# TAMUparametric/PPOPT

Measured on AMD Instinct MI355X. Metric: candidate active-sets checked/sec (combinatorial mpQP), higher is better.
Workload: dtype f64

## Files before the change

ppopt_amd/csrc/kernels.hpp:

```cpp
#pragma once
#include <stdint.h>

#include "kkt.hpp"
#include "records.hpp"

#ifndef MPC_GLOBAL
#define MPC_GLOBAL __global__
#define MPC_LB(...) __launch_bounds__(__VA_ARGS__)
#endif

namespace mpc {

constexpr int ST_INFEASIBLE = 0, ST_FEASIBLE = 1, ST_OPT_NO_REGION = 2, ST_REGION = 3, ST_SINGULAR = 4, ST_LP_LIMIT = 5;
constexpr int ST_OPT_PENDING = 6;
constexpr int ST_RETRY = 7;
constexpr int ST_NEEDX = 8;
constexpr int ST_NEEDX_SING = 9;
static_assert(ST_REGION == SLOT_ST_REGION, "records.hpp: the status of a slot that carries a record");
constexpr double ZERO_ROW_ATOL = 1e-8;
constexpr double FULL_DIM_RADIUS = 1e-8;

struct DevProblem {
    int n_x, n_t, n_c, n_eq, n_tc, is_qp, kkt_mode;
    const double *A, *b, *F, *c, *H, *Q, *A_t, *b_t;
// ... 552 lines not shown
    if (lane == 63) wsum[w] = incl;
    __syncthreads();
    if (w == 0) {
        int t = lane < 16 ? wsum[lane] : 0, ti = t;
#pragma unroll
        for (int off = 1; off < 16; off <<= 1) { const int o = __shfl_up(ti, off); if (lane >= off) ti += o; }
        if (lane < 16) wsum[lane] = ti - t;
        if (lane == 15 && total_out) *total_out = ti;
    }
    __syncthreads();
    return incl - v + wsum[w];
}
constexpr int SCAN_IT = 4;
__device__ __forceinline__ void block_exclusive_scan_it(const int (&v)[SCAN_IT], int (&ex)[SCAN_IT], int *total_out) {
    constexpr int NW = 16 / SCAN_IT;
    __shared__ int wsum_it[NW];
    const int lane = threadIdx.x & 63, w = threadIdx.x >> 6;
    int s = 0;
#pragma unroll
    for (int k = 0; k < SCAN_IT; ++k) s += v[k];
    int incl = s;
#pragma unroll
    for (int off = 1; off < 64; off <<= 1) { const int o = __shfl_up(incl, off); if (lane >= off) incl += o; }
    if (lane == 63) wsum_it[w] = incl;
    __syncthreads();
    int base = 0;
#pragma unroll
    for (int k = 0; k < NW; ++k) base += k < w ? wsum_it[k] : 0;
    if (total_out && threadIdx.x == 64 * NW - 1) *total_out = base + incl;
    int run = base + incl - s;
#pragma unroll
    for (int k = 0; k < SCAN_IT; ++k) { ex[k] = run; run += v[k]; }
    __syncthreads();
}
MPC_GLOBAL void MPC_LB(1024 / SCAN_IT) k_scan_block_sums(const int32_t *__restrict__ in, long long n, int32_t *__restrict__ sums) {
    __shared__ int tot;
    const long long i0 = blockIdx.x * (long long)SCAN_BLOCK + (long long)threadIdx.x * SCAN_IT;
    int v[SCAN_IT], ex[SCAN_IT];
#pragma unroll
    for (int k = 0; k < SCAN_IT; ++k) v[k] = i0 + k < n ? in[i0 + k] : 0;
    block_exclusive_scan_it(v, ex, &tot);
    if (threadIdx.x == 0) sums[blockIdx.x] = tot;
}
MPC_GLOBAL void MPC_LB(1024 / SCAN_IT) k_scan_sums(int32_t *__restrict__ sums, int nb, int32_t *__restrict__ total) {
    __shared__ int tot;
    int carry = 0;
    for (int base = 0; base < nb; base += SCAN_BLOCK) {
        const int i0 = base + (int)threadIdx.x * SCAN_IT;
        int v[SCAN_IT], ex[SCAN_IT];
#pragma unroll
        for (int k = 0; k < SCAN_IT; ++k) v[k] = i0 + k < nb ? sums[i0 + k] : 0;
        block_exclusive_scan_it(v, ex, &tot);
#pragma unroll
        for (int k = 0; k < SCAN_IT; ++k) if (i0 + k < nb) sums[i0 + k] = ex[k] + carry;
        carry += tot;
        __syncthreads();
    }
    if (threadIdx.x == 0) *total = carry;
}
MPC_GLOBAL void MPC_LB(1024 / SCAN_IT) k_scan_apply(const int32_t *__restrict__ in, int32_t *__restrict__ out, long long n,
                                                    const int32_t *__restrict__ sums) {
    const long long i0 = blockIdx.x * (long long)SCAN_BLOCK + (long long)threadIdx.x * SCAN_IT;
    int v[SCAN_IT], ex[SCAN_IT];
#pragma unroll
    for (int k = 0; k < SCAN_IT; ++k) v[k] = i0 + k < n ? in[i0 + k] : 0;
    block_exclusive_scan_it(v, ex, nullptr);
    const int add = sums[blockIdx.x];
#pragma unroll
    for (int k = 0; k < SCAN_IT; ++k) if (i0 + k < n) out[i0 + k] = ex[k] + add;
}

constexpr int PART_CLASSES = 4;
__device__ __forceinline__ int part_class(unsigned long long spec, int st) { return (int)((spec >> (4 * (st & 15))) & 15ull); }
MPC_GLOBAL void MPC_LB(1024 / SCAN_IT) k_part_count(const uint8_t *__restrict__ status, long long n, unsigned long long spec,
                                                     int32_t *__restrict__ blockcounts, int nb) {
    constexpr int BT = 1024 / SCAN_IT, NW = BT / 64;
    __shared__ int wc[16][PART_CLASSES];
    const int wave = threadIdx.x >> 6, lane = threadIdx.x & 63;
#pragma unroll
    for (int j = 0; j < SCAN_IT; ++j) {
        const long long i = blockIdx.x * 1024LL + j * BT + threadIdx.x;
        const int cls = i < n ? part_class(spec, status[i]) : 15;
#pragma unroll
        for (int c = 0; c < PART_CLASSES; ++c) {
            const unsigned long long m = __ballot(cls == c);
            if (lane == 0) wc[j * NW + wave][c] = __popcll(m);
        }
    }
    __syncthreads();
    if (threadIdx.x < PART_CLASSES) {
        int tot = 0;
        for (int w = 0; w < 16; ++w) tot += wc[w][threadIdx.x];
        blockcounts[threadIdx.x * nb + blockIdx.x] = tot;
    }
}
MPC_GLOBAL void MPC_LB(1024 / SCAN_IT) k_part_sums(int32_t *__restrict__ blockcounts, int nb, int32_t *__restrict__ totals) {
    __shared__ int tot;
    int32_t *sums = blockcounts + (size_t)blockIdx.x * nb;
    int carry = 0;
    for (int base = 0; base < nb; base += SCAN_BLOCK) {
        const int i0 = base + (int)threadIdx.x * SCAN_IT;
        int v[SCAN_IT], ex[SCAN_IT];
#pragma unroll
        for (int k = 0; k < SCAN_IT; ++k) v[k] = i0 + k < nb ? sums[i0 + k] : 0;
        block_exclusive_scan_it(v, ex, &tot);
#pragma unroll
        for (int k = 0; k < SCAN_IT; ++k) if (i0 + k < nb) sums[i0 + k] = ex[k] + carry;
        carry += tot;
        __syncthreads();
    }
    if (threadIdx.x == 0) totals[blockIdx.x] = carry;
}
MPC_GLOBAL void MPC_LB(1024 / SCAN_IT) k_part_scatter(const uint8_t *__restrict__ status, long long n, unsigned long long spec,
                                                       const int32_t *__restrict__ blockbase, int nb, int32_t *__restrict__ lists) {
    constexpr int BT = 1024 / SCAN_IT, NW = BT / 64;
    __shared__ int wc[16][PART_CLASSES];
    const int wave = threadIdx.x >> 6, lane = threadIdx.x & 63;
    int cls[SCAN_IT], within[SCAN_IT];
#pragma unroll
    for (int j = 0; j < SCAN_IT; ++j) {
        const long long i = blockIdx.x * 1024LL + j * BT + threadIdx.x;
        cls[j] = i < n ? part_class(spec, status[i]) : 15;
        within[j] = 0;
#pragma unroll
        for (int c = 0; c < PART_CLASSES; ++c) {
            const unsigned long long m = __ballot(cls[j] == c);
            if (lane == 0) wc[j * NW + wave][c] = __popcll(m);
            if (cls[j] == c) within[j] = __popcll(m & ((1ull << lane) - 1ull));
        }
    }
    __syncthreads();
#pragma unroll
    for (int j = 0; j < SCAN_IT; ++j) {
        if (cls[j] < PART_CLASSES) {
            const long long i = blockIdx.x * 1024LL + j * BT + threadIdx.x;
            int before = 0;
            for (int w = 0; w < j * NW + wave; ++w) before += wc[w][cls[j]];
            lists[(size_t)cls[j] * n + blockbase[cls[j] * nb + blockIdx.x] + before + within[j]] = (int32_t)i;
        }
    }
}

MPC_GLOBAL void k_flag_status(const uint8_t *__restrict__ status, long long n, int lo, int hi, int32_t *__restrict__ flag) {
    const long long i = blockIdx.x * (long long)blockDim.x + threadIdx.x;
    if (i < n) flag[i] = status[i] >= lo && status[i] <= hi;
}
MPC_GLOBAL void k_scatter_index(const int32_t *__restrict__ flag, const int32_t *__restrict__ pos, long long n,
                                int32_t *__restrict__ list) {
    const long long i = blockIdx.x * (long long)blockDim.x + threadIdx.x;
    if (i < n && flag[i]) list[pos[i]] = (int32_t)i;
}

struct ZeroBufs { void *p[4]; unsigned long long bytes[4]; };
MPC_GLOBAL void MPC_LB(256) k_zero_bufs(ZeroBufs z) {
    for (int j = 0; j < 4; ++j) {
        const unsigned long long bytes = z.bytes[j];
        if (!z.p[j] || bytes == 0) continue;
        if ((reinterpret_cast<unsigned long long>(z.p[j]) & 7ull) == 0 && (bytes & 7ull) == 0) {
            unsigned long long *p = reinterpret_cast<unsigned long long *>(z.p[j]);
            for (unsigned long long i = blockIdx.x * 256ull + threadIdx.x; i < bytes / 8; i += (unsigned long long)gridDim.x * 256ull) p[i] = 0ull;
        } else {
            unsigned char *p = reinterpret_cast<unsigned char *>(z.p[j]);
            for (unsigned long long i = blockIdx.x * 256ull + threadIdx.x; i < bytes; i += (unsigned long long)gridDim.x * 256ull) p[i] = 0;
        }
    }
}

struct RegionPrep { ZeroBufs z; const int32_t *copy_src; int32_t *copy_dst; long long copy_n; int32_t *head_i; int fi, first, extra; };
MPC_GLOBAL void MPC_LB(256) k_region_prep(RegionPrep a) {
    for (int j = 0; j < 4; ++j) {
        const unsigned long long bytes = a.z.bytes[j];
        if (!a.z.p[j] || bytes == 0) continue;
        if ((reinterpret_cast<unsigned long long>(a.z.p[j]) & 7ull) == 0 && (bytes & 7ull) == 0) {
            unsigned long long *p = reinterpret_cast<unsigned long long *>(a.z.p[j]);
            for (unsigned long long i = blockIdx.x * 256ull + threadIdx.x; i < bytes / 8; i += (unsigned long long)gridDim.x * 256ull) p[i] = 0ull;
        } else {
            unsigned char *p = reinterpret_cast<unsigned char *>(a.z.p[j]);
            for (unsigned long long i = blockIdx.x * 256ull + threadIdx.x; i < bytes; i += (unsigned long long)gridDim.x * 256ull) p[i] = 0;
        }
    }
    for (long long i = blockIdx.x * 256ll + threadIdx.x; i < a.copy_n; i += (long long)gridDim.x * 256ll) a.copy_dst[i] = a.copy_src[i];
    for (int j = blockIdx.x * 256 + threadIdx.x; j < a.extra; j += gridDim.x * 256) { int32_t *hi = a.head_i + (size_t)(a.first + j) * a.fi; hi[SW_STATUS] = 0; hi[SW_CAND] = -1; }
}

struct FetchCopy { const void *src[3]; void *dst[3]; unsigned long long bytes[3]; unsigned int *counter; int32_t *flag; };
MPC_GLOBAL void MPC_LB(256) k_fetch_slots(FetchCopy a) {
    for (int j = 0; j < 3; ++j) {
        const unsigned long long words = a.bytes[j] / 4;
        const unsigned int *src = static_cast<const unsigned int *>(a.src[j]);
        unsigned int *dst = static_cast<unsigned int *>(a.dst[j]);
        for (unsigned long long i = blockIdx.x * 256ull + threadIdx.x; i < words; i += (unsigned long long)gridDim.x * 256ull) dst[i] = src[i];
    }
    __builtin_amdgcn_fence(__ATOMIC_RELEASE, "");
    __syncthreads();
    if (threadIdx.x == 0) {
        if (atomicAdd(a.counter, 1u) + 1u == gridDim.x) {
            __builtin_amdgcn_fence(__ATOMIC_ACQ_REL, "");
            atomicExch(a.counter, 0u);
            __hip_atomic_store(a.flag, 1, __ATOMIC_RELEASE, __HIP_MEMORY_SCOPE_SYSTEM);
        }
    }
}

struct FetchEntry { const void *src; void *dst; unsigned long long bytes; };
MPC_GLOBAL void MPC_LB(256) k_fetch_many(const FetchEntry *__restrict__ tab) {
    const FetchEntry e = tab[blockIdx.y];
    const unsigned long long words = e.bytes / 4;
    const unsigned int *src = static_cast<const unsigned int *>(e.src);
    unsigned int *dst = static_cast<unsigned int *>(e.dst);
    for (unsigned long long i = blockIdx.x * 256ull + threadIdx.x; i < words; i += (unsigned long long)gridDim.x * 256ull) dst[i] = src[i];
}

MPC_GLOBAL void k_publish_words(const unsigned int *__restrict__ src, unsigned int *__restrict__ dst, int n) {
    for (int i = threadIdx.x; i < n; i += blockDim.x) dst[i] = src[i];
}
MPC_GLOBAL void k_publish_words2(const unsigned int *__restrict__ src1, int n1, const unsigned int *__restrict__ src2, int n2, unsigned int *__restrict__ dst) {
    for (int i = threadIdx.x; i < n1 + n2; i += blockDim.x) dst[i] = i < n1 ? src1[i] : src2[i - n1];
}

constexpr int SMALL_LEVEL_N = 16384;
MPC_GLOBAL void MPC_LB(1024) k_compact_small(const uint8_t *__restrict__ status, int n, int lo, int hi,
                                                        int32_t *__restrict__ list, int32_t *__restrict__ total) {
    __shared__ int wc[16];
    __shared__ int base;
    const int wave = threadIdx.x >> 6, lane = threadIdx.x & 63;
    if (threadIdx.x == 0) base = 0;
    __syncthreads();
    for (int start = 0; start < n; start += 1024) {
        const int i = start + (int)threadIdx.x;
        const bool f = i < n && status[i] >= lo && status[i] <= hi;
        const unsigned long long m = __ballot(f);
        if (lane == 0) wc[wave] = __popcll(m);
        __syncthreads();
        int before = base;
        for (int w = 0; w < wave; ++w) before += wc[w];
        if (f) list[before + __popcll(m & ((1ull << lane) - 1ull))] = i;
        __syncthreads();
        if (threadIdx.x == 0) { int t = 0; for (int w = 0; w < 16; ++w) t += wc[w]; base += t; }
        __syncthreads();
    }
    if (threadIdx.x == 0) *total = base;
}
MPC_GLOBAL void MPC_LB(1024) k_partition_small(const uint8_t *__restrict__ status, int n, unsigned long long spec,
                                                          int32_t *__restrict__ lists, long long stride, int32_t *__restrict__ totals) {
    __shared__ int wc[16][PART_CLASSES];
    __shared__ int base[PART_CLASSES];
    const int wave = threadIdx.x >> 6, lane = threadIdx.x & 63;
    if (threadIdx.x < PART_CLASSES) base[threadIdx.x] = 0;
    __syncthreads();
    for (int start = 0; start < n; start += 1024) {
        const int i = start + (int)threadIdx.x;
        const int cls = i < n ? part_class(spec, status[i]) : 15;
        int within = 0;
#pragma unroll
        for (int c = 0; c < PART_CLASSES; ++c) {
            const unsigned long long m = __ballot(cls == c);
            if (lane == 0) wc[wave][c] = __popcll(m);
            if (cls == c) within = __popcll(m & ((1ull << lane) - 1ull));
        }
        __syncthreads();
        if (cls < PART_CLASSES) {
            int before = base[cls];
            for (int w = 0; w < wave; ++w) before += wc[w][cls];
            lists[(size_t)cls * stride + before + within] = i;
        }
        __syncthreads();
        if (threadIdx.x < PART_CLASSES) { int t = 0; for (int w = 0; w < 16; ++w) t += wc[w][threadIdx.x]; base[threadIdx.x] += t; }
        __syncthreads();
    }
    if (threadIdx.x < PART_CLASSES) totals[threadIdx.x] = base[threadIdx.x];
}
MPC_GLOBAL void MPC_LB(1024) k_scan_small(const int32_t *__restrict__ in, int32_t *__restrict__ out, int n,
                                                     int32_t *__restrict__ total) {
    __shared__ int tot;
    int carry = 0;
    for (int start = 0; start < n; start += SCAN_BLOCK) {
        const int i = start + (int)threadIdx.x;
        const int ex = block_exclusive_scan_1024(i < n ? in[i] : 0, &tot);
        __syncthreads();
        if (i < n) out[i] = ex + carry;
        carry += tot;
        __syncthreads();
    }
    if (threadIdx.x == 0) *total = carry;
}

constexpr int EXPAND_LOWDIM = 1, EXPAND_PENDING = 2;
__device__ __forceinline__ bool expands(int st, int keep_lowdim = 0) {
    return st == ST_FEASIBLE || st == ST_REGION || st == ST_SINGULAR || st == ST_LP_LIMIT || ((keep_lowdim & EXPAND_LOWDIM) && st == ST_OPT_NO_REGION) ||
           ((keep_lowdim & EXPAND_PENDING) && st == ST_OPT_PENDING);
}

template <int MW>
__device__ __forceinline__ void set_mask(const int32_t *as, int k, unsigned long long (&p)[MW]) {
#pragma unroll
    for (int w = 0; w < MW; ++w) p[w] = 0;
    for (int i = 0; i < k; ++i) {
        const int v = as[i];
#pragma unroll
        for (int w = 0; w < MW; ++w) if ((v >> 6) == w) p[w] |= 1ull << (v & 63);
    }
}

template <int MW>
MPC_GLOBAL void MPC_LB(64) k_children_count(DevProblem P, const int32_t *__restrict__ cands, long long n, int k,
                                                       const uint8_t *__restrict__ status,
                                                       const unsigned long long *__restrict__ pruned, long long n_pruned,
                                                       unsigned long long *__restrict__ childmask, int32_t *__restrict__ count, int keep_lowdim) {
    const long long c = blockIdx.x;
    const int lane = lane_id();
    if (c >= n) return;
    const int st = status[c];
    unsigned long long m[MW];
#pragma unroll
    for (int w = 0; w < MW; ++w) m[w] = 0;
    if (expands(st, keep_lowdim)) {
        const int32_t *as = cands + (size_t)c * k;
        unsigned long long p[MW], a[MW], kill[MW];
        set_mask<MW>(as, k, p);
        const int start = k > 0 ? as[k - 1] + 1 : 0;
        int stop = P.n_c;
        if (!P.is_qp && st == ST_FEASIBLE) stop = min(stop, (k + 1) + P.n_c - P.n_x);
#pragma unroll
        for (int w = 0; w < MW; ++w) {
            const int lo = max(start - 64 * w, 0), hi = min(stop - 64 * w, 64);
            a[w] = hi > lo ? ((hi >= 64 ? ~0ull : ((1ull << hi) - 1ull)) & ~((1ull << lo) - 1ull)) : 0ull;
            kill[w] = 0;
        }
        for (long long j = lane; j < n_pruned; j += 64) {
            unsigned long long d[MW];
            int bits = 0;
#pragma unroll
            for (int w = 0; w < MW; ++w) { d[w] = pruned[MW * j + w] & ~p[w]; bits += __popcll(d[w]); }
            if (bits == 0) {
#pragma unroll
                for (int w = 0; w < MW; ++w) kill[w] = ~0ull;
            } else if (bits == 1) {
#pragma unroll
                for (int w = 0; w < MW; ++w) kill[w] |= d[w];
            }
        }
#pragma unroll
        for (int w = 0; w < MW; ++w) {
            for (int off = 32; off > 0; off >>= 1) kill[w] |= __shfl_xor(kill[w], off);
            m[w] = a[w] & ~kill[w];
        }
    }
    if (lane == 0) {
        int cnt = 0;
#pragma unroll
        for (int w = 0; w < MW; ++w) { childmask[MW * c + w] = m[w]; cnt += __popcll(m[w]); }
        count[c] = cnt;
    }
}

constexpr int PB_OFF = 256, PB_CUR = 513, PB_SINGLES = 776, PB_WORDS = PB_SINGLES + 2 * 4;
template <int MW>
__device__ __forceinline__ int pruned_min_member(const unsigned long long *p, int ne, int *n_members) {
    int first = -1, cnt = 0;
#pragma unroll
    for (int w = 0; w < MW; ++w) {
        unsigned long long v = p[w];
        const int lo = ne - 64 * w;
        if (lo >= 64) v = 0ull; else if (lo > 0) v &= ~((1ull << lo) - 1ull);
        cnt += __popcll(v);
        if (first < 0 && v) first = 64 * w + __ffsll((long long)v) - 1;
    }
    *n_members = cnt;
    return first;
}
template <int MW>
MPC_GLOBAL void MPC_LB(256) k_pruned_bucket_count(const unsigned long long *__restrict__ pruned, long long n_pruned, int ne, int32_t *__restrict__ head) {
    const long long j = (long long)blockIdx.x * 256 + threadIdx.x;
    if (j >= n_pruned) return;
    int cnt = 0;
    const int b = pruned_min_member<MW>(pruned + (size_t)MW * j, ne, &cnt);
    if (cnt <= 1) {
        unsigned long long *singles = reinterpret_cast<unsigned long long *>(head + PB_SINGLES);
#pragma unroll
        for (int w = 0; w < MW; ++w) { const unsigned long long v = cnt == 0 ? ~0ull : pruned[(size_t)MW * j + w]; if (v) atomicOr(&singles[w], v); }
    } else if (b >= 0) atomicAdd(&head[b], 1);
}
MPC_GLOBAL void MPC_LB(256) k_pruned_bucket_scan(int32_t *__restrict__ head) {
    __shared__ int sh[256];
    const int t = threadIdx.x;
    sh[t] = head[t];
    __syncthreads();
    for (int off = 1; off < 256; off <<= 1) { const int v = t >= off ? sh[t - off] : 0; __syncthreads(); sh[t] += v; __syncthreads(); }
    head[PB_OFF + t + 1] = sh[t];
    if (t == 0) head[PB_OFF] = 0;
    head[PB_CUR + t] = 0;
}
template <int MW>
MPC_GLOBAL void MPC_LB(256) k_pruned_bucket_scatter(const unsigned long long *__restrict__ pruned, long long n_pruned, int ne, int32_t *__restrict__ head,
                                                            unsigned long long *__restrict__ out) {
    const long long j = (long long)blockIdx.x * 256 + threadIdx.x;
    if (j >= n_pruned) return;
    int cnt = 0;
    const int b = pruned_min_member<MW>(pruned + (size_t)MW * j, ne, &cnt);
    if (cnt <= 1 || b < 0) return;
    const int pos = head[PB_OFF + b] + atomicAdd(&head[PB_CUR + b], 1);
#pragma unroll
    for (int w = 0; w < MW; ++w) out[(size_t)MW * pos + w] = pruned[(size_t)MW * j + w];
}
template <int MW>
MPC_GLOBAL void MPC_LB(64) k_children_count_b(DevProblem P, const int32_t *__restrict__ cands, long long n, int k,
                                                         const uint8_t *__restrict__ status,
                                                         const unsigned long long *__restrict__ bucketed, const int32_t *__restrict__ head,
                                                         unsigned long long *__restrict__ childmask, int32_t *__restrict__ count, int keep_lowdim) {
    const long long c = blockIdx.x;
    const int lane = lane_id();
    if (c >= n) return;
    const int st = status[c];
    unsigned long long m[MW];
#pragma unroll
    for (int w = 0; w < MW; ++w) m[w] = 0;
    if (expands(st, keep_lowdim)) {
        const int32_t *as = cands + (size_t)c * k;
        unsigned long long p[MW], a[MW], kill[MW];
        set_mask<MW>(as, k, p);
        const int start = k > 0 ? as[k - 1] + 1 : 0;
        int stop = P.n_c;
        if (!P.is_qp && st == ST_FEASIBLE) stop = min(stop, (k + 1) + P.n_c - P.n_x);
        const unsigned long long *singles = reinterpret_cast<const unsigned long long *>(head + PB_SINGLES);
#pragma unroll
        for (int w = 0; w < MW; ++w) {
            const int lo = max(start - 64 * w, 0), hi = min(stop - 64 * w, 64);
            a[w] = hi > lo ? ((hi >= 64 ? ~0ull : ((1ull << hi) - 1ull)) & ~((1ull << lo) - 1ull)) : 0ull;
            kill[w] = singles[w] & ~p[w];
            const int lo_e = P.n_eq - 64 * w;
            const unsigned long long emask = lo_e >= 64 ? ~0ull : (lo_e > 0 ? ((1ull << lo_e) - 1ull) : 0ull);
            if (singles[w] & p[w] & ~emask) kill[w] = ~0ull;
        }
        for (int mi = P.n_eq; mi < k; ++mi) {
            const int b = as[mi];
            const int j0 = head[PB_OFF + b], j1 = head[PB_OFF + b + 1];
            for (int j = j0 + lane; j < j1; j += 64) {
                unsigned long long d[MW];
                int bits = 0;
#pragma unroll
                for (int w = 0; w < MW; ++w) { d[w] = bucketed[(size_t)MW * j + w] & ~p[w]; bits += __popcll(d[w]); }
                if (bits == 0) {
#pragma unroll
                    for (int w = 0; w < MW; ++w) kill[w] = ~0ull;
                } else if (bits == 1) {
#pragma unroll
                    for (int w = 0; w < MW; ++w) kill[w] |= d[w];
                }
            }
        }
#pragma unroll
        for (int w = 0; w < MW; ++w) {
            for (int off = 32; off > 0; off >>= 1) kill[w] |= __shfl_xor(kill[w], off);
            m[w] = a[w] & ~kill[w];
        }
    }
    if (lane == 0) {
        int cnt = 0;
#pragma unroll
        for (int w = 0; w < MW; ++w) { childmask[MW * c + w] = m[w]; cnt += __popcll(m[w]); }
        count[c] = cnt;
    }
}

MPC_GLOBAL void MPC_LB(64) k_children_write(const int32_t *__restrict__ cands, long long n, int k, int mw,
                                                       const unsigned long long *__restrict__ childmask,
                                                       const int32_t *__restrict__ offset, int32_t *__restrict__ out,
                                                       const uint8_t *__restrict__ stored, int32_t *__restrict__ parent_slot) {
    const long long c = blockIdx.x;
    const int lane = lane_id();
    if (c >= n) return;
    const int32_t *as = cands + (size_t)c * k;
    int base = offset[c];
    const int ps = (stored && stored[c]) ? (int)c : -1;
    for (int half = 0; half < mw; ++half) {
        const unsigned long long mk = childmask[(size_t)mw * c + half];
        if (!mk) continue;
        const bool mine = (mk >> lane) & 1ull;
        const int pos = base + __popcll(mk & ((1ull << lane) - 1ull));
        if (mine) {
            int32_t *o = out + (size_t)pos * (k + 1);
            for (int i = 0; i < k; ++i) o[i] = as[i];
            o[k] = half * 64 + lane;
            if (parent_slot) parent_slot[pos] = ps;
        }
        base += __popcll(mk);
    }
}

template <int MW>
MPC_GLOBAL void k_pruned_append(const int32_t *__restrict__ cands, long long n, int k, const uint8_t *__restrict__ status,
                                unsigned long long *__restrict__ out, LevelCounters *ctr, int keep_lowdim) {
    constexpr int PER = 16;
    __shared__ unsigned int wsum[4], base_s;
    const long long c0 = (long long)blockIdx.x * 256 * PER;
    if (c0 >= n) return;
    const int lane = threadIdx.x & 63, wave = threadIdx.x >> 6;
    unsigned int bits = 0;
#pragma unroll
    for (int j = 0; j < PER; ++j) {
        const long long c = c0 + (long long)j * 256 + threadIdx.x;
        const int st = c < n ? status[c] : 0;
        if (c < n && (st == ST_INFEASIBLE || (st == ST_OPT_NO_REGION && !keep_lowdim))) bits |= 1u << j;
    }
    const unsigned int cnt = (unsigned int)__popc(bits);
    unsigned int incl = cnt;
#pragma unroll
    for (int off = 1; off < 64; off <<= 1) { const unsigned int o = (unsigned int)__shfl_up((int)incl, off); if (lane >= off) incl += o; }
    if (lane == 63) wsum[wave] = incl;
    __syncthreads();
    if (threadIdx.x == 0) {
        const unsigned int total = wsum[0] + wsum[1] + wsum[2] + wsum[3];
        base_s = total ? atomicAdd(&ctr->n_pruned_new, total) : 0u;
    }
    __syncthreads();
    unsigned int pos = base_s + incl - cnt;
    for (int w = 0; w < wave; ++w) pos += wsum[w];
    while (bits) {
        const int j = __builtin_ctz(bits);
        bits &= bits - 1;
        const long long c = c0 + (long long)j * 256 + threadIdx.x;
        unsigned long long p[MW];
        set_mask<MW>(cands + (size_t)c * k, k, p);
#pragma unroll
        for (int w = 0; w < MW; ++w) out[MW * (size_t)pos + w] = p[w];
        ++pos;
    }
}

__device__ __forceinline__ unsigned int load_word_agent(const unsigned int *p) { return __hip_atomic_load(p, __ATOMIC_RELAXED, __HIP_MEMORY_SCOPE_AGENT); }
template <int MW>
MPC_GLOBAL void MPC_LB(1024) k_small_end(const int32_t *__restrict__ cands, int n, int k, const uint8_t *__restrict__ status,
                                         unsigned long long *__restrict__ pruned_out, LevelCounters *ctr, int keep_lowdim,
                                         int32_t *__restrict__ n_retry, int32_t *__restrict__ n_late,
                                         const unsigned int *pub_src2, int pub_n2, unsigned int *pub_dst) {
    __shared__ unsigned int hist[16];
    const int lane = threadIdx.x & 63;
    if (threadIdx.x < 16) hist[threadIdx.x] = 0;
    __syncthreads();
    for (int start = 0; start < n; start += 1024) {
        const int i = start + (int)threadIdx.x;
        const int st = i < n ? status[i] : 15;
#pragma unroll
        for (int b = 0; b < 12; ++b) {
            const unsigned long long m = __ballot(st == b);
            if (lane == 0 && m) atomicAdd(&hist[b], (unsigned int)__popcll(m));
        }
        const bool cut = st == ST_INFEASIBLE || (st == ST_OPT_NO_REGION && !keep_lowdim);
        const unsigned long long mc = __ballot(cut);
        if (mc) {
            unsigned int base = 0;
            if (lane == 0) base = atomicAdd(&ctr->n_pruned_new, (unsigned int)__popcll(mc));
            base = (unsigned int)__builtin_amdgcn_readfirstlane((int)base);
            if (cut) {
                unsigned long long pm[MW];
                set_mask<MW>(cands + (size_t)i * k, k, pm);
                const size_t pos = base + (unsigned int)__popcll(mc & ((1ull << lane) - 1ull));
#pragma unroll
                for (int w = 0; w < MW; ++w) pruned_out[MW * pos + w] = pm[w];
            }
        }
    }
    __syncthreads();
    if (threadIdx.x < 8) {
        const unsigned int v = hist[threadIdx.x] + (threadIdx.x < 4 ? hist[threadIdx.x + 8] : 0u);
        if (v) atomicAdd(&ctr->status[threadIdx.x], (unsigned long long)v);
    }
    if (threadIdx.x == 0) { *n_retry = (int32_t)hist[7];    *n_late = (int32_t)hist[ST_OPT_PENDING]; }
    if (pub_dst) {
        __threadfence();
        __syncthreads();
        const unsigned int *src1 = reinterpret_cast<const unsigned int *>(ctr);
        const int n1 = (int)(sizeof(LevelCounters) / 4);
        for (int i = threadIdx.x; i < n1 + pub_n2; i += 1024) pub_dst[i] = load_word_agent(i < n1 ? src1 + i : pub_src2 + (i - n1));
    }
}
MPC_GLOBAL void MPC_LB(1024) k_scan_publish(const int32_t *__restrict__ in, int32_t *__restrict__ out, int n, int32_t *total,
                                            const unsigned int *src1, int n1, const unsigned int *src2, int n2, unsigned int *dst) {
    __shared__ int tot;
    int carry = 0;
    for (int start = 0; start < n; start += SCAN_BLOCK) {
        const int i = start + (int)threadIdx.x;
        const int ex = block_exclusive_scan_1024(i < n ? in[i] : 0, &tot);
        __syncthreads();
        if (i < n) out[i] = ex + carry;
        carry += tot;
        __syncthreads();
    }
    if (threadIdx.x == 0) *total = carry;
    __threadfence();
    __syncthreads();
    for (int i = threadIdx.x; i < n1 + n2; i += 1024) dst[i] = load_word_agent(i < n1 ? src1 + i : src2 + (i - n1));
}

constexpr int RRETRY_MERGE_MAX = 1024;
struct RretryMerge {
    const int32_t *opt_list; const int32_t *rlist; const uint8_t *status; const double *recd; const int32_t *reci;
    double *headd; int32_t *headi; double *epool;
    RecordShape sh;
    int n_opt, n_rretry, row0;
};
MPC_GLOBAL void MPC_LB(256) k_rretry_merge(RretryMerge a) {
    __shared__ int slots[RRETRY_MERGE_MAX], src[RRETRY_MERGE_MAX], rowoff[RRETRY_MERGE_MAX];
    __shared__ int wc[4];
    __shared__ int m;
    const int tid = threadIdx.x, lane = tid & 63, wave = tid >> 6;
    const RecordShape &sh = a.sh;
    const int fd = sh.fd(), fi = sh.fi(), rec_d = (int)sh.rec_d(), rec_i = (int)sh.rec_i(), nt = sh.nt, nr = sh.row_len();
    if (tid == 0) m = 0;
    __syncthreads();
    for (int start = 0; start < a.n_opt; start += 256) {
        const int w = start + tid;
        const bool f = w < a.n_opt && a.headi[(size_t)w * fi + SW_STATUS] == ST_RETRY;
        const unsigned long long mk = __ballot(f);
        if (lane == 0) wc[wave] = __popcll(mk);
        __syncthreads();
        int before = m;
        for (int v = 0; v < wave; ++v) before += wc[v];
        const int pos = before + __popcll(mk & ((1ull << lane) - 1ull));
        if (f && pos < RRETRY_MERGE_MAX) slots[pos] = w;
        __syncthreads();
        if (tid == 0) m += wc[0] + wc[1] + wc[2] + wc[3];
        __syncthreads();
    }
    const int mm = min(m, RRETRY_MERGE_MAX);
    for (int j = tid; j < mm; j += 256) {
        const int cand = a.opt_list[slots[j]];
        int r = -1;
        for (int q = 0; q < a.n_rretry; ++q) if (a.rlist[q] == cand) { r = q; break; }
        src[j] = r;
        rowoff[j] = (r >= 0 && a.status[cand] == ST_REGION) ? a.reci[(size_t)r * rec_i + FW_NE] : 0;
    }
    __syncthreads();
    if (tid == 0) { int run = a.row0; for (int j = 0; j < mm; ++j) { const int ne = rowoff[j]; rowoff[j] = run; run += ne; } }
    __syncthreads();
    for (int j = 0; j < mm; ++j) {
        const int w = slots[j], cand = a.opt_list[w], r = src[j];
        const int st = a.status[cand];
        int32_t *oi = a.headi + (size_t)w * fi;
        double *od = a.headd + (size_t)w * fd;
        for (int i = tid; i < fi; i += 256) oi[i] = i == SW_STATUS ? st : (i == SW_CAND ? cand : (i < SW_LISTS ? 0 : -1));
        if (r < 0 || st != ST_REGION) continue;
        for (int i = tid; i < fd; i += 256) od[i] = 0.0;
        __syncthreads();
        const double *rd = a.recd + (size_t)r * rec_d;
        const int32_t *ri = a.reci + (size_t)r * rec_i;
        const int kk = ri[FW_K], nE = ri[FW_NE], n_om = ri[FW_NOM], n_la = ri[FW_NLA], n_re = ri[FW_NRE];
        const double *Al = rd + sh.f_Al(), *bl = rd + sh.f_bl(), *E = rd + sh.f_E(), *f = rd + sh.f_f();
        for (int i = tid; i < sh.law(); i += 256) od[i] = rd[i];
        for (int i = tid; i < kk * nt; i += 256) od[sh.s_Al() + i] = Al[i];
        for (int i = tid; i < kk; i += 256) od[sh.s_bl() + i] = bl[i];
        if (tid == 0) { oi[SW_NE] = nE; oi[SW_NOM] = n_om; oi[SW_NLA] = n_la; oi[SW_NRE] = n_re; oi[SW_ROW0] = rowoff[j]; }
        int32_t *act = oi + sh.s_act(), *om = oi + sh.s_om(), *la = oi + sh.s_la(), *ridx = oi + sh.s_ridx(), *rcon = oi + sh.s_rcon();
        for (int i = tid; i < kk; i += 256) act[i] = ri[sh.f_act() + i];
        for (int i = tid; i < n_om; i += 256) om[i] = ri[sh.f_om() + i];
        for (int i = tid; i < n_la; i += 256) la[i] = ri[sh.f_la() + i];
        for (int i = tid; i < n_re; i += 256) { ridx[i] = ri[sh.f_ridx() + i]; rcon[i] = ri[sh.f_rcon() + i]; }
        for (int i = tid; i < nE * nr; i += 256) {
            const int rr = i / nr, t = i - rr * nr;
            a.epool[(size_t)(rowoff[j] + rr) * nr + t] = t == 0 ? f[rr] : E[(size_t)rr * nt + (t - 1)];
        }
        __syncthreads();
    }
}

MPC_GLOBAL void k_close_open(const int32_t *__restrict__ list, int n_list, uint8_t *__restrict__ status) {
    const int w = blockIdx.x * blockDim.x + threadIdx.x;
    if (w < n_list) { const int c = list[w]; status[c] = (uint8_t)(status[c] == 9 ? ST_SINGULAR : ST_FEASIBLE); }
}

MPC_GLOBAL void k_apply_status(const int32_t *__restrict__ list, int n_list, const uint8_t *__restrict__ tmp, uint8_t *__restrict__ status) {
    const int w = blockIdx.x * blockDim.x + threadIdx.x;
    if (w < n_list) { const int c = list[w]; status[c] = tmp[c]; }
}

MPC_GLOBAL void k_init_slots(int32_t *__restrict__ head_i, int fi, int first, int count, int st, const int32_t *__restrict__ list) {
    const int j = blockIdx.x * blockDim.x + threadIdx.x;
    if (j < count) { int32_t *hi = head_i + (size_t)(first + j) * fi; hi[SW_STATUS] = st; hi[SW_CAND] = list ? list[j] : -1; }
}
MPC_GLOBAL void k_take_rows(const int32_t *__restrict__ src, long long n_new, int width, long long start, long long stride,
                            int32_t *__restrict__ dst) {
    const long long idx = (long long)blockIdx.x * blockDim.x + threadIdx.x;
    if (idx >= n_new * width) return;
    const long long r = idx / width;
    dst[idx] = src[(start + r * stride) * width + (idx - r * width)];
}

MPC_GLOBAL void k_base_frontier(int n_eq, int32_t *out) { for (int i = threadIdx.x; i < n_eq; i += blockDim.x) out[i] = i; }
MPC_GLOBAL void k_root_frontier(int n_eq, int n_c, int32_t *out) {
    const int i = blockIdx.x * blockDim.x + threadIdx.x;
    const int cnt = n_c - n_eq;
    if (i >= cnt) return;
    int32_t *o = out + (size_t)i * (n_eq + 1);
    for (int j = 0; j < n_eq; ++j) o[j] = j;
    o[n_eq] = n_eq + i;
}

}
```

Before: 325.9 million.

## Batch candidate loads via readlane and keep several pruned loads in flight in children kernels

Each wave now loads the candidate's active-set indices once, coalesced across lanes, and broadcasts them with readlane instead of every lane reading all k indices serially. The pruned-set scan issues CH_FLIGHT loads per lane before culling, to raise memory-level parallelism. In the bucketed variant the per-member bucket loops are flattened into one combined index space so lanes stay busy across short buckets. The child-write kernel replaces per-half serial copying with broadcast values written by all owning lanes. This adds index-mapping arithmetic and clamped redundant loads at tails, and the write kernel hardcodes up to 4 mask words.

```diff
diff --git a/ppopt_amd/csrc/kernels.hpp b/ppopt_amd/csrc/kernels.hpp
--- a/ppopt_amd/csrc/kernels.hpp
+++ b/ppopt_amd/csrc/kernels.hpp
@@ -878,6 +878,73 @@
     }
 }
 
+__device__ __forceinline__ int members_chunk(const int32_t *as, int k, int base, int lane) { return base + lane < k ? as[base + lane] : -1; }
+__device__ __forceinline__ unsigned long long readlane64(unsigned long long v, int l) {
+    return ((unsigned long long)(unsigned int)__builtin_amdgcn_readlane((int)(v >> 32), l) << 32) | (unsigned int)__builtin_amdgcn_readlane((int)v, l);
+}
+template <int MW>
+__device__ __forceinline__ int parent_mask(const int32_t *as, int k, int lane, int v0, unsigned long long (&p)[MW]) {
+#pragma unroll
+    for (int w = 0; w < MW; ++w) p[w] = 0;
+    int last = -1;
+    for (int base = 0; base < k; base += 64) {
+        const int v = base ? members_chunk(as, k, base, lane) : v0;
+        const int nn = min(k - base, 64);
+        for (int i = 0; i < nn; ++i) {
+            last = __builtin_amdgcn_readlane(v, i);
+#pragma unroll
+            for (int w = 0; w < MW; ++w) if ((last >> 6) == w) p[w] |= 1ull << (last & 63);
+        }
+    }
+    return last;
+}
+template <int MW>
+__device__ __forceinline__ void allowed_children(const DevProblem &P, int st, int k, int last, unsigned long long (&a)[MW]) {
+    const int start = last + 1;
+    int stop = P.n_c;
+    if (!P.is_qp && st == ST_FEASIBLE) stop = min(stop, (k + 1) + P.n_c - P.n_x);
+#pragma unroll
+    for (int w = 0; w < MW; ++w) {
+        const int lo = max(start - 64 * w, 0), hi = min(stop - 64 * w, 64);
+        a[w] = hi > lo ? ((hi >= 64 ? ~0ull : ((1ull << hi) - 1ull)) & ~((1ull << lo) - 1ull)) : 0ull;
+    }
+}
+template <int MW>
+__device__ __forceinline__ void cull(const unsigned long long (&e)[MW], const unsigned long long (&p)[MW], unsigned long long (&kill)[MW]) {
+    unsigned long long d[MW];
+    int bits = 0;
+#pragma unroll
+    for (int w = 0; w < MW; ++w) { d[w] = e[w] & ~p[w]; bits += __popcll(d[w]); }
+    if (bits == 0) {
+#pragma unroll
+        for (int w = 0; w < MW; ++w) kill[w] = ~0ull;
+    } else if (bits == 1) {
+#pragma unroll
+        for (int w = 0; w < MW; ++w) kill[w] |= d[w];
+    }
+}
+template <int MW>
+__device__ __forceinline__ void children_store(long long c, int lane, bool live, const unsigned long long (&a)[MW], unsigned long long (&kill)[MW],
+                                               unsigned long long *__restrict__ childmask, int32_t *__restrict__ count) {
+    unsigned long long m[MW];
+#pragma unroll
+    for (int w = 0; w < MW; ++w) m[w] = 0;
+    if (live) {
+#pragma unroll
+        for (int w = 0; w < MW; ++w) {
+            for (int off = 32; off > 0; off >>= 1) kill[w] |= __shfl_xor(kill[w], off);
+            m[w] = a[w] & ~kill[w];
+        }
+    }
+    if (lane == 0) {
+        int cnt = 0;
+#pragma unroll
+        for (int w = 0; w < MW; ++w) { childmask[MW * c + w] = m[w]; cnt += __popcll(m[w]); }
+        count[c] = cnt;
+    }
+}
+constexpr int CH_FLIGHT = 4;
+
 template <int MW>
 MPC_GLOBAL void MPC_LB(64) k_children_count(DevProblem P, const int32_t *__restrict__ cands, long long n, int k,
                                                        const uint8_t *__restrict__ status,
@@ -886,48 +953,29 @@
     const long long c = blockIdx.x;
     const int lane = lane_id();
     if (c >= n) return;
+    const int32_t *as = cands + (size_t)c * k;
+    const int v0 = members_chunk(as, k, 0, lane);
     const int st = status[c];
-    unsigned long long m[MW];
-#pragma unroll
-    for (int w = 0; w < MW; ++w) m[w] = 0;
-    if (expands(st, keep_lowdim)) {
-        const int32_t *as = cands + (size_t)c * k;
-        unsigned long long p[MW], a[MW], kill[MW];
-        set_mask<MW>(as, k, p);
-        const int start = k > 0 ? as[k - 1] + 1 : 0;
-        int stop = P.n_c;
-        if (!P.is_qp && st == ST_FEASIBLE) stop = min(stop, (k + 1) + P.n_c - P.n_x);
-#pragma unroll
-        for (int w = 0; w < MW; ++w) {
-            const int lo = max(start - 64 * w, 0), hi = min(stop - 64 * w, 64);
-            a[w] = hi > lo ? ((hi >= 64 ? ~0ull : ((1ull << hi) - 1ull)) & ~((1ull << lo) - 1ull)) : 0ull;
-            kill[w] = 0;
-        }
-        for (long long j = lane; j < n_pruned; j += 64) {
-            unsigned long long d[MW];
-            int bits = 0;
-#pragma unroll
-            for (int w = 0; w < MW; ++w) { d[w] = pruned[MW * j + w] & ~p[w]; bits += __popcll(d[w]); }
-            if (bits == 0) {
-#pragma unroll
-                for (int w = 0; w < MW; ++w) kill[w] = ~0ull;
-            } else if (bits == 1) {
-#pragma unroll
-                for (int w = 0; w < MW; ++w) kill[w] |= d[w];
+    unsigned long long p[MW], a[MW], kill[MW];
+    const int last = parent_mask<MW>(as, k, lane, v0, p);
+    const bool live = expands(st, keep_lowdim);
+#pragma unroll
+    for (int w = 0; w < MW; ++w) a[w] = kill[w] = 0;
+    if (live) {
+        allowed_children<MW>(P, st, k, last, a);
+        for (long long j0 = 0; j0 < n_pruned; j0 += 64 * CH_FLIGHT) {
+            unsigned long long e[CH_FLIGHT][MW];
+#pragma unroll
+            for (int u = 0; u < CH_FLIGHT; ++u) {
+                const long long j = min(j0 + 64 * u + lane, n_pruned - 1);
+#pragma unroll
+                for (int w = 0; w < MW; ++w) e[u][w] = pruned[MW * j + w];
             }
-        }
-#pragma unroll
-        for (int w = 0; w < MW; ++w) {
-            for (int off = 32; off > 0; off >>= 1) kill[w] |= __shfl_xor(kill[w], off);
-            m[w] = a[w] & ~kill[w];
-        }
-    }
-    if (lane == 0) {
-        int cnt = 0;
-#pragma unroll
-        for (int w = 0; w < MW; ++w) { childmask[MW * c + w] = m[w]; cnt += __popcll(m[w]); }
-        count[c] = cnt;
-    }
+#pragma unroll
+            for (int u = 0; u < CH_FLIGHT; ++u) cull<MW>(e[u], p, kill);
+        }
+    }
+    children_store<MW>(c, lane, live, a, kill, childmask, count);
 }
 
 constexpr int PB_OFF = 256, PB_CUR = 513, PB_SINGLES = 776, PB_WORDS = PB_SINGLES + 2 * 4;
@@ -987,56 +1035,55 @@
     const long long c = blockIdx.x;
     const int lane = lane_id();
     if (c >= n) return;
+    const int32_t *as = cands + (size_t)c * k;
+    const unsigned long long *singles = reinterpret_cast<const unsigned long long *>(head + PB_SINGLES);
+    const int v0 = members_chunk(as, k, 0, lane);
+    const unsigned long long sv = lane < MW ? singles[lane] : 0ull;
     const int st = status[c];
-    unsigned long long m[MW];
-#pragma unroll
-    for (int w = 0; w < MW; ++w) m[w] = 0;
-    if (expands(st, keep_lowdim)) {
-        const int32_t *as = cands + (size_t)c * k;
-        unsigned long long p[MW], a[MW], kill[MW];
-        set_mask<MW>(as, k, p);
-        const int start = k > 0 ? as[k - 1] + 1 : 0;
-        int stop = P.n_c;
-        if (!P.is_qp && st == ST_FEASIBLE) stop = min(stop, (k + 1) + P.n_c - P.n_x);
-        const unsigned long long *singles = reinterpret_cast<const unsigned long long *>(head + PB_SINGLES);
-#pragma unroll
-        for (int w = 0; w < MW; ++w) {
-            const int lo = max(start - 64 * w, 0), hi = min(stop - 64 * w, 64);
-            a[w] = hi > lo ? ((hi >= 64 ? ~0ull : ((1ull << hi) - 1ull)) & ~((1ull << lo) - 1ull)) : 0ull;
-            kill[w] = singles[w] & ~p[w];
-            const int lo_e = P.n_eq - 64 * w;
-            const unsigned long long emask = lo_e >= 64 ? ~0ull : (lo_e > 0 ? ((1ull << lo_e) - 1ull) : 0ull);
-            if (singles[w] & p[w] & ~emask) kill[w] = ~0ull;
-        }
-        for (int mi = P.n_eq; mi < k; ++mi) {
-            const int b = as[mi];
-            const int j0 = head[PB_OFF + b], j1 = head[PB_OFF + b + 1];
-            for (int j = j0 + lane; j < j1; j += 64) {
-                unsigned long long d[MW];
-                int bits = 0;
-#pragma unroll
-                for (int w = 0; w < MW; ++w) { d[w] = bucketed[(size_t)MW * j + w] & ~p[w]; bits += __popcll(d[w]); }
-                if (bits == 0) {
-#pragma unroll
-                    for (int w = 0; w < MW; ++w) kill[w] = ~0ull;
-                } else if (bits == 1) {
-#pragma unroll
-                    for (int w = 0; w < MW; ++w) kill[w] |= d[w];
+    unsigned long long p[MW], a[MW], kill[MW];
+    const int last = parent_mask<MW>(as, k, lane, v0, p);
+    const bool live = expands(st, keep_lowdim);
+#pragma unroll
+    for (int w = 0; w < MW; ++w) {
+        const unsigned long long s = readlane64(sv, w);
+        a[w] = 0;
+        kill[w] = s & ~p[w];
+        const int lo_e = P.n_eq - 64 * w;
+        const unsigned long long emask = lo_e >= 64 ? ~0ull : (lo_e > 0 ? ((1ull << lo_e) - 1ull) : 0ull);
+        if (s & p[w] & ~emask) kill[w] = ~0ull;
+    }
+    if (live) {
+        allowed_children<MW>(P, st, k, last, a);
+        for (int base = 0; base < k; base += 64) {
+            const int v = base ? members_chunk(as, k, base, lane) : v0;
+            const int i_lo = max(P.n_eq - base, 0), i_hi = min(k - base, 64);
+            int j0 = 0, len = 0;
+            if (lane >= i_lo && lane < i_hi) { j0 = head[PB_OFF + v]; len = head[PB_OFF + v + 1] - j0; }
+            int T = 0;
+            for (int i = i_lo; i < i_hi; ++i) T += __builtin_amdgcn_readlane(len, i);
+            for (int t0 = 0; t0 < T; t0 += 64 * CH_FLIGHT) {
+                int t[CH_FLIGHT], src[CH_FLIGHT];
+#pragma unroll
+                for (int u = 0; u < CH_FLIGHT; ++u) { t[u] = min(t0 + 64 * u + lane, T - 1); src[u] = 0; }
+                int e_i = 0;
+                for (int i = i_lo; i < i_hi; ++i) {
+                    const int d_i = __builtin_amdgcn_readlane(j0, i) - e_i;
+#pragma unroll
+                    for (int u = 0; u < CH_FLIGHT; ++u) if (t[u] >= e_i) src[u] = t[u] + d_i;
+                    e_i += __builtin_amdgcn_readlane(len, i);
                 }
+                unsigned long long e[CH_FLIGHT][MW];
+#pragma unroll
+                for (int u = 0; u < CH_FLIGHT; ++u) {
+#pragma unroll
+                    for (int w = 0; w < MW; ++w) e[u][w] = bucketed[(size_t)MW * src[u] + w];
+                }
+#pragma unroll
+                for (int u = 0; u < CH_FLIGHT; ++u) cull<MW>(e[u], p, kill);
             }
         }
-#pragma unroll
-        for (int w = 0; w < MW; ++w) {
-            for (int off = 32; off > 0; off >>= 1) kill[w] |= __shfl_xor(kill[w], off);
-            m[w] = a[w] & ~kill[w];
-        }
-    }
-    if (lane == 0) {
-        int cnt = 0;
-#pragma unroll
-        for (int w = 0; w < MW; ++w) { childmask[MW * c + w] = m[w]; cnt += __popcll(m[w]); }
-        count[c] = cnt;
-    }
+    }
+    children_store<MW>(c, lane, live, a, kill, childmask, count);
 }
 
 MPC_GLOBAL void MPC_LB(64) k_children_write(const int32_t *__restrict__ cands, long long n, int k, int mw,
@@ -1047,20 +1094,35 @@
     const int lane = lane_id();
     if (c >= n) return;
     const int32_t *as = cands + (size_t)c * k;
-    int base = offset[c];
+    const int v0 = members_chunk(as, k, 0, lane);
+    unsigned long long mk[4];
+#pragma unroll
+    for (int half = 0; half < 4; ++half) mk[half] = childmask[(size_t)mw * c + min(half, mw - 1)];
+    int first = offset[c];
+#pragma unroll
+    for (int half = 1; half < 4; ++half) if (half >= mw) mk[half] = 0ull;
     const int ps = (stored && stored[c]) ? (int)c : -1;
-    for (int half = 0; half < mw; ++half) {
-        const unsigned long long mk = childmask[(size_t)mw * c + half];
-        if (!mk) continue;
-        const bool mine = (mk >> lane) & 1ull;
-        const int pos = base + __popcll(mk & ((1ull << lane) - 1ull));
-        if (mine) {
-            int32_t *o = out + (size_t)pos * (k + 1);
-            for (int i = 0; i < k; ++i) o[i] = as[i];
-            o[k] = half * 64 + lane;
-            if (parent_slot) parent_slot[pos] = ps;
-        }
-        base += __popcll(mk);
+    int pos[4];
+#pragma unroll
+    for (int half = 0; half < 4; ++half) {
+        pos[half] = ((mk[half] >> lane) & 1ull) ? first + __popcll(mk[half] & ((1ull << lane) - 1ull)) : -1;
+        first += __popcll(mk[half]);
+    }
+    for (int base = 0; base < k; base += 64) {
+        const int v = base ? members_chunk(as, k, base, lane) : v0;
+        const int nn = min(k - base, 64);
+        for (int i = 0; i < nn; ++i) {
+            const int a_i = __builtin_amdgcn_readlane(v, i);
+#pragma unroll
+            for (int half = 0; half < 4; ++half) if (pos[half] >= 0) out[(size_t)pos[half] * (k + 1) + base + i] = a_i;
+        }
+    }
+#pragma unroll
+    for (int half = 0; half < 4; ++half) {
+        if (pos[half] >= 0) {
+            out[(size_t)pos[half] * (k + 1) + k] = half * 64 + lane;
+            if (parent_slot) parent_slot[pos[half]] = ps;
+        }
     }
 }
 
```

Result: slower. 309.9 million (-4.9%).
